# bcgsc/ntSynt

Measured on AMD Instinct MI355X. Metric: minimizer-sketch Gbases/s (sketch with common Bloom filter, inputs resident in HBM), higher is better.
Workload: dtype u64

## Files before the change

ntsynt_amd/csrc/nts_microbench.inc:

```
constexpr int VB_CHAINS = 8;
constexpr int VB_UNROLL = 4;

enum ValuKind
{
  VK_XOR_B32 = 0,
  VK_ALIGNBIT_B32 = 1,
  VK_LSHL_ADD_U64 = 2,
  VK_LSHLREV_B64 = 3,
  VK_MUL_LO_U32 = 4,
  VK_MAD_U64_U32 = 5,
  VK_ADD_CO_PAIR = 6,
  VK_XOR_DEPENDENT = 7,
  VK_ADD3_U32 = 8,
  VK_CMP_ADDC = 9,
  VK_ROLL31_STEP = 10,
  VK_COUNT = 11
};

template <int KIND>
__global__ __launch_bounds__(256) void k_valu_bench(uint32_t iters, unsigned long long* __restrict__ cycles, uint32_t* __restrict__ sink)
{
  uint32_t a[VB_CHAINS];
  uint64_t q[VB_CHAINS];
  const uint32_t seed = threadIdx.x * 2654435761u + blockIdx.x;
#pragma unroll
  for (int c = 0; c < VB_CHAINS; ++c) {
    a[c] = seed + 0x9E3779B9u * (c + 1);
    q[c] = ((uint64_t)a[c] << 32) | (a[c] ^ 0x5bd1e995u);
  }
  const uint32_t b = seed | 1u;
  uint32_t pen = 0;
  const uint64_t b64 = ((uint64_t)b << 20) | 3u;
  __syncthreads();
  const uint64_t t0 = __builtin_amdgcn_s_memtime();
  for (uint32_t it = 0; it < iters; ++it) {
#pragma unroll
    for (int u = 0; u < VB_UNROLL; ++u) {
#pragma unroll
      for (int c = 0; c < VB_CHAINS; ++c) {
        if constexpr (KIND == VK_XOR_B32) asm volatile("v_xor_b32 %0, %1, %0" : "+v"(a[c]) : "v"(b));
        if constexpr (KIND == VK_ALIGNBIT_B32) asm volatile("v_alignbit_b32 %0, %0, %1, 7" : "+v"(a[c]) : "v"(b));
        if constexpr (KIND == VK_LSHL_ADD_U64) asm volatile("v_lshl_add_u64 %0, %0, 1, %1" : "+v"(q[c]) : "v"(b64));
        if constexpr (KIND == VK_LSHLREV_B64) asm volatile("v_lshlrev_b64 %0, 1, %0" : "+v"(q[c]));
        if constexpr (KIND == VK_MUL_LO_U32) asm volatile("v_mul_lo_u32 %0, %0, %1" : "+v"(a[c]) : "v"(b));
        if constexpr (KIND == VK_MAD_U64_U32) asm volatile("v_mad_u64_u32 %0, vcc, %1, %1, %0" : "+v"(q[c]) : "v"(b) : "vcc");
        if constexpr (KIND == VK_ADD_CO_PAIR) {
          uint32_t lo = (uint32_t)q[c], hi = (uint32_t)(q[c] >> 32);
          asm volatile("v_add_co_u32 %0, vcc, %0, %2\n\tv_addc_co_u32 %1, vcc, %1, %2, vcc" : "+v"(lo), "+v"(hi) : "v"(b) : "vcc");
          q[c] = ((uint64_t)hi << 32) | lo;
        }
        if constexpr (KIND == VK_XOR_DEPENDENT) asm volatile("v_xor_b32 %0, %1, %0" : "+v"(a[0]) : "v"(b));
        if constexpr (KIND == VK_ADD3_U32) asm volatile("v_add3_u32 %0, %0, %1, 2" : "+v"(a[c]) : "v"(b));
        if constexpr (KIND == VK_CMP_ADDC)
          asm volatile("v_cmp_ge_u32 vcc, %1, %0\n\tv_addc_co_u32 %0, vcc, %0, %0, vcc" : "+v"(a[c]) : "s"(iters) : "vcc");
        if constexpr (KIND == VK_ROLL31_STEP) {
          uint32_t& wf = a[c & ~1];
          uint32_t& wr = a[c | 1];
          uint32_t s3, t1, x;
          asm volatile("v_add3_u32 %3, %0, %1, 2\n\t"
                       "v_cmp_ge_u32 vcc, %7, %3\n\t"
                       "v_addc_co_u32 %2, vcc, %2, %2, vcc\n\t"
                       "v_lshlrev_b32 %4, 1, %0\n\t"
                       "v_alignbit_b32 %0, %0, %4, 31\n\t"
                       "v_xor_b32 %0, %0, %6\n\t"
                       "v_xor_b32 %5, %1, %6\n\t"
                       "v_lshrrev_b32 %4, 1, %5\n\t"
                       "v_alignbit_b32 %1, %4, %5, 1"
                       : "+v"(wf), "+v"(wr), "+v"(pen), "=&v"(s3), "=&v"(t1), "=&v"(x)
                       : "v"(b), "s"(iters)
                       : "vcc");
        }
      }
    }
  }
  const uint64_t t1 = __builtin_amdgcn_s_memtime();
  uint32_t acc = 0;
#pragma unroll
  for (int c = 0; c < VB_CHAINS; ++c) acc ^= a[c] ^ (uint32_t)q[c] ^ (uint32_t)(q[c] >> 32);
  acc ^= pen;
  if (acc == 0x12345678u) sink[0] = acc;
  if ((threadIdx.x & 63) == 0) cycles[(uint64_t)blockIdx.x * (blockDim.x / 64) + threadIdx.x / 64] = t1 - t0;
}

typedef void (*ValuBenchFn)(uint32_t, unsigned long long*, uint32_t*);
static ValuBenchFn valu_bench_fn(int kind)
{
  switch (kind) {
    case VK_XOR_B32: return k_valu_bench<VK_XOR_B32>;
    case VK_ALIGNBIT_B32: return k_valu_bench<VK_ALIGNBIT_B32>;
    case VK_LSHL_ADD_U64: return k_valu_bench<VK_LSHL_ADD_U64>;
    case VK_LSHLREV_B64: return k_valu_bench<VK_LSHLREV_B64>;
    case VK_MUL_LO_U32: return k_valu_bench<VK_MUL_LO_U32>;
    case VK_MAD_U64_U32: return k_valu_bench<VK_MAD_U64_U32>;
    case VK_ADD_CO_PAIR: return k_valu_bench<VK_ADD_CO_PAIR>;
    case VK_XOR_DEPENDENT: return k_valu_bench<VK_XOR_DEPENDENT>;
    case VK_ADD3_U32: return k_valu_bench<VK_ADD3_U32>;
    case VK_CMP_ADDC: return k_valu_bench<VK_CMP_ADDC>;
    case VK_ROLL31_STEP: return k_valu_bench<VK_ROLL31_STEP>;
  }
  return nullptr;
}
```

ntsynt_amd/csrc/nts_pruned.inc:

```
constexpr uint32_t SEL_CAP = 2048;
constexpr uint32_t SEL_PER_LANE = 64;
constexpr uint32_t SEL_TILE = HASH_THREADS * SEL_PER_LANE;
constexpr uint32_t SPARSE_THREADS = 256;
constexpr uint32_t SPARSE_ITEMS = 2;
constexpr uint32_t SPARSE_BLOCK = SPARSE_THREADS * SPARSE_ITEMS;
constexpr uint32_t CC_TILES = 8;

struct SelParams
{
  const uint8_t* code;
  const uint32_t* pack;
  const uint64_t* run_pos;
  const uint64_t* run_vstart;
  uint32_t n_runs;
  uint64_t n_valid;
  HashParams hp;
  const uint32_t* bf;
  FastMod fm;
  uint64_t tau;
  uint32_t flush_at;
  uint64_t* seg_j;
  uint64_t* seg_key;
  uint64_t seg_cap;
  unsigned long long* seg_count;
// ... 261 lines not shown
    {
      const uint32_t lane = tid & 63u;
      unsigned long long todo = __ballot(shared_lane);
      while (todo) {
        const uint32_t o = (uint32_t)__ffsll((long long)todo) - 1u;
        todo &= todo - 1ULL;
        const uint64_t jo = __shfl(j_lane, (int)o, 64);
        const uint32_t nm = __shfl(n_mine, (int)o, 64);
        const uint32_t run_o = __shfl(run, (int)o, 64);
        const uint32_t cur_o = __shfl(cur, (int)o, 64);
        bool hit = false;
        uint64_t h = 0;
        if (lane < nm) {
          const uint64_t j = jo + lane;
          uint32_t rr = run_o;
          while (P.run_vstart[rr + 1] <= j) ++rr;
          const uint64_t s0 = P.run_pos[rr] + (j - P.run_vstart[rr]);
          uint64_t hf = 0, hr = 0;
          hash_init(P.hp, [&](uint32_t i) { return base_abs(s0 + i); }, hf, hr);
          h = hf + hr;
          hit = (uint32_t)(h >> 32) <= tau_hi;
        }
        const unsigned long long hm = __ballot(hit);
        if (hit) {
          const uint32_t rank = (uint32_t)__popcll(hm & ((1ULL << lane) - 1ULL));
          const uint32_t spare_o = SEL_SLOTS * ROW + (tid - lane + o) * 8u;
          *reinterpret_cast<uint64_t*>(ch_bytes + min(cur_o + rank * ROW, spare_o)) = h;
        }
        if (lane == o) {
          cur += (uint32_t)__popcll(hm) * ROW;
          pen_lo |= (uint32_t)hm;
          pen_hi |= (uint32_t)(hm >> 32);
        }
      }
    }
    if (!over) flush();
    if (!__syncthreads_or(over)) {
      static_assert(SEL_SLOTS * HASH_THREADS >= SEL_CAP, "the general path stages SEL_CAP candidates in the same arrays");
      uint32_t accepted = 0;
      const uint32_t off = block_excl_scan_256(acc, s_w, &accepted);
      if (tid == 0) {
        s_base = accepted ? atomicAdd(&P.seg_count[seg], (unsigned long long)accepted) : 0ULL;
        P.tile_off[tile] = s_base;
        P.tile_cnt[tile] = accepted;
        P.tile_ordered[tile] = 1;
      }
      __syncthreads();
      const uint64_t base = s_base;
      if (accepted == 0 || base + accepted > P.seg_cap) return;
      uint64_t* dj = P.seg_j + (uint64_t)seg * P.seg_cap + base + off;
      uint64_t* dk = P.seg_key + (uint64_t)seg * P.seg_cap + base + off;
      for (uint32_t i = 0; i < acc; ++i) {
        dj[i] = J0 + first + (uint32_t)__builtin_ctzll(acc_mask);
        acc_mask &= acc_mask - 1;
        dk[i] = s_ch[i * HASH_THREADS + tid];
      }
      return;
    }
  }
  if (tid == 0) P.tile_ordered[tile] = 0;
  roll_pass(0, SEL_TILE);
  __syncthreads();
  const uint32_t total = s_ctl[0];
  if (total <= SEL_CAP) {
    uint32_t mine = 0, accepted = 0;
    const uint32_t bits = probe_staged(total, &mine);
    (void)block_excl_scan_256(mine, s_w, &accepted);
    if (tid == 0) {
      s_base = accepted ? atomicAdd(&P.seg_count[seg], (unsigned long long)accepted) : 0ULL;
      P.tile_off[tile] = s_base;
      P.tile_cnt[tile] = accepted;
    }
    __syncthreads();
    const uint64_t base = s_base;
    if (accepted == 0 || base + accepted > P.seg_cap) return;
    write_staged(total, bits, (uint64_t)seg * P.seg_cap + base);
    return;
  }
  constexpr uint32_t RANGE = 2048;
  uint32_t accepted = 0;
  for (uint32_t r0 = 0; r0 < SEL_TILE; r0 += RANGE) {
    __syncthreads();
    if (tid == 0) s_ctl[0] = 0;
    __syncthreads();
    roll_pass(r0, r0 + RANGE);
    __syncthreads();
    uint32_t mine = 0, acc = 0;
    (void)probe_staged(s_ctl[0], &mine);
    (void)block_excl_scan_256(mine, s_w, &acc);
    accepted += acc;
  }
  if (tid == 0) {
    s_base = accepted ? atomicAdd(&P.seg_count[seg], (unsigned long long)accepted) : 0ULL;
    P.tile_off[tile] = s_base;
    P.tile_cnt[tile] = accepted;
    s_ctl[1] = 0;
  }
  __syncthreads();
  const uint64_t base = s_base;
  if (accepted == 0 || base + accepted > P.seg_cap) return;
  for (uint32_t r0 = 0; r0 < SEL_TILE; r0 += RANGE) {
    __syncthreads();
    if (tid == 0) s_ctl[0] = 0;
    __syncthreads();
    roll_pass(r0, r0 + RANGE);
    __syncthreads();
    uint32_t mine = 0;
    const uint32_t n = s_ctl[0];
    const uint32_t bits = probe_staged(n, &mine);
    write_staged(n, bits, (uint64_t)seg * P.seg_cap + base);
  }
}

constexpr uint32_t HIW_TILE = 64 * SEL_PER_LANE;
constexpr uint32_t HIW_WAVES = 8;
constexpr uint32_t HIW_THREADS = 64 * HIW_WAVES;
constexpr uint32_t HIW_PER_MAX = 4;
constexpr uint32_t HI_K_MAX = 32;

__device__ __forceinline__ uint32_t hi_wform(uint64_t h)
{
  const uint32_t hi = (uint32_t)(h >> 32);
  return (hi & ~1u) | (hi >> 31);
}

__device__ __forceinline__ uint64_t sload64(const uint64_t* p, uint32_t idx)
{
  uint64_t v;
  asm volatile("s_load_dwordx2 %0, %1, %2\n\ts_waitcnt lgkmcnt(0)" : "=&s"(v) : "s"(p), "s"(idx * 8u) : "memory");
  return v;
}

__device__ __forceinline__ uint32_t wave_excl_scan_small(uint32_t v, uint64_t below, uint32_t* total)
{
  uint32_t pre = 0, tot = 0;
#pragma unroll
  for (uint32_t b = 0; b < 3; ++b) {
    const unsigned long long m = __ballot((v >> b) & 1u);
    pre += (uint32_t)__popcll(m & below) << b;
    tot += (uint32_t)__popcll(m) << b;
  }
  if (__ballot(v >> 3) != 0ULL) {
#pragma unroll
    for (uint32_t b = 3; b < 7; ++b) {
      const unsigned long long m = __ballot((v >> b) & 1u);
      pre += (uint32_t)__popcll(m & below) << b;
      tot += (uint32_t)__popcll(m) << b;
    }
  }
  *total = tot;
  return pre;
}

__device__ __forceinline__ void hi_roll64(const uint32_t (&ro)[5], const uint32_t (&ri)[5], uint32_t sh_o, uint32_t sh_i, const ulonglong2* s_T,
                                          const uint2* s_roll, uint32_t nch, uint32_t limit, uint32_t& pen0, uint32_t& pen1)
{
  uint32_t O[4], I[4];
#pragma unroll
  for (int q = 0; q < 4; ++q) {
    O[q] = __builtin_amdgcn_alignbit(ro[q + 1], ro[q], sh_o);
    I[q] = __builtin_amdgcn_alignbit(ri[q + 1], ri[q], sh_i);
  }
  uint32_t wf = 0, wr = 0;
#pragma unroll
  for (uint32_t c = 0; c < HI_K_MAX / 4; ++c) {
    if (c < nch) {
      const ulonglong2 e = s_T[c * 256u + ((O[c >> 2] >> (8u * (c & 3u))) & 255u)];
      wf ^= (uint32_t)(e.x >> 32);
      wr ^= (uint32_t)(e.y >> 32);
    }
  }
  wf = (wf & ~1u) | (wf >> 31);
  wr = (wr & ~1u) | (wr >> 31);
  const uint8_t* const roll_bytes = reinterpret_cast<const uint8_t*>(s_roll);
  pen0 = pen1 = 0;
#pragma unroll
  for (int q = 0; q < 4; ++q) {
    const uint32_t even = (O[q] & 0x33333333u) | ((I[q] & 0x33333333u) << 2);
    const uint32_t odd = ((O[q] >> 2) & 0x33333333u) | (I[q] & 0xCCCCCCCCu);
    uint32_t pen = 0;
#pragma unroll
    for (int j0 = 0; j0 < 16; j0 += 8) {
      uint2 tb[8];
#pragma unroll
      for (int jj = 0; jj < 8; ++jj) {
        const int j = j0 + jj;
        const uint32_t pairs = (j & 1) ? odd : even;
        const int sh = 4 * (j >> 1) - 3;
        const uint32_t t8 = (sh < 0 ? pairs << 3 : pairs >> sh) & 0x78u;
        tb[jj] = *reinterpret_cast<const uint2*>(roll_bytes + t8);
      }
#pragma unroll
      for (int jj = 0; jj < 8; ++jj) {
        const uint32_t s = wf + wr + 2u;
        asm("v_cmp_ge_u32 vcc, %2, %1\n\tv_addc_co_u32 %0, vcc, %0, %0, vcc" : "+v"(pen) : "v"(s), "s"(limit) : "vcc");
        wf = __builtin_amdgcn_alignbit(wf, wf << 1, 31) ^ tb[jj].x;
        const uint32_t x = wr ^ tb[jj].y;
        wr = __builtin_amdgcn_alignbit(x >> 1, x, 1);
      }
    }
    const uint32_t nat = __brev(pen) >> 16;
    if (q < 2)
      pen0 |= nat << (16 * q);
    else
      pen1 |= nat << (16 * (q - 2));
  }
}

__device__ __forceinline__ uint2 hi_roll_multirun(const uint32_t* pack, const uint64_t* run_pos, const uint64_t* run_vstart, uint32_t n_runs,
                                               uint32_t run_lo, uint64_t j_lane, uint32_t n_mine, uint32_t k, const ulonglong2* s_T,
                                               const uint2* s_roll, uint32_t nch, uint32_t limit, bool& straddles)
{
  uint32_t rl = run_lo, rh = n_runs;
  while (rh - rl > 1) {
    const uint32_t mid = rl + ((rh - rl) >> 1);
    if (run_vstart[mid] <= j_lane)
      rl = mid;
    else
      rh = mid;
  }
  uint32_t pen0, pen1;
  straddles = false;
  if (n_mine == SEL_PER_LANE && j_lane + SEL_PER_LANE <= run_vstart[rl + 1]) {
    const uint64_t xo = run_pos[rl] + (j_lane - run_vstart[rl]);
    const uint32_t* wo = pack + (xo >> 4);
    const uint32_t* wi = pack + ((xo + k) >> 4);
    uint32_t ro[5], ri[5];
#pragma unroll
    for (int q = 0; q < 5; ++q) {
      ro[q] = wo[q];
      ri[q] = wi[q];
    }
    hi_roll64(ro, ri, 2u * ((uint32_t)xo & 15u), 2u * ((uint32_t)(xo + k) & 15u), s_T, s_roll, nch, limit, pen0, pen1);
  } else {
    pen0 = pen1 = 0;
    straddles = true;
  }
  return make_uint2(pen0, pen1);
}

constexpr uint32_t HIW_STAGE_WORDS = 272;
constexpr uint32_t ELIM_REACH = 6;

template <bool HAS_BF, uint32_t HIW_PER>
__global__ __launch_bounds__(HIW_THREADS) void k_hash_select_hi(SelParams P, uint32_t nch, uint32_t tpw, uint64_t n_tiles)
{
  constexpr uint32_t HIW_LIST = 64 * HIW_PER;
  static_assert(HIW_PER == 2 || HIW_PER == 4, "the waits count the probes");
  extern __shared__ __align__(16) uint8_t hi_dyn_lds[];
  ulonglong2* const s_T = reinterpret_cast<ulonglong2*>(hi_dyn_lds);
  __shared__ uint2 s_roll[16];
  __shared__ __align__(16) uint32_t s_stage[HIW_WAVES][2][HIW_STAGE_WORDS];
  __shared__ uint16_t s_lists[HIW_WAVES][HIW_LIST];
  __shared__ __align__(16) uint32_t s_probe[HIW_WAVES][HIW_PER][64];
  const uint32_t tid = threadIdx.x, lane = tid & 63u;
  const uint32_t wv = __builtin_amdgcn_readfirstlane(tid >> 6);
  {
    const ulonglong2* src = reinterpret_cast<const ulonglong2*>(P.hp.init4);
    for (uint32_t i = tid; i < nch * 256u; i += HIW_THREADS) s_T[i] = src[i];
  }
  if (tid < 16) s_roll[tid] = make_uint2(hi_wform(P.hp.roll_f[tid]), hi_wform(P.hp.roll_r[tid]));
  __syncthreads();
  uint16_t* const s_list = s_lists[wv];
  const uint32_t stage_lds = (uint32_t)(uintptr_t)(__attribute__((address_space(3))) uint32_t*)(&s_stage[wv][0][0]);
  const uint32_t probe_lds = (uint32_t)(uintptr_t)(__attribute__((address_space(3))) uint32_t*)(&s_probe[wv][0][0]);
  const uint32_t k = P.hp.k;
  const uint32_t tau_hi = (uint32_t)(P.tau >> 32);
  const uint32_t limit = 2u * (tau_hi >> 1) + 4u;
  const uint32_t key16_shift = 48u - (uint32_t)__builtin_clzll(P.tau | 0x10000ULL);
  const uint32_t blk = (blockIdx.x & 1u) ? gridDim.x - 1u - (blockIdx.x >> 1) : (blockIdx.x >> 1);
  const uint64_t tile_first = ((uint64_t)blk * HIW_WAVES + wv) * tpw;
  if (tile_first >= n_tiles) return;
  const uint32_t my_tiles = (uint32_t)min((uint64_t)tpw, n_tiles - tile_first);
  const uint32_t first = SEL_PER_LANE * lane;
  const uint64_t below = (1ULL << lane) - 1ULL;

  uint32_t run_next = 0;
  {
    const uint64_t J0 = tile_first * HIW_TILE;
    uint32_t lo = 0, hi = P.n_runs;
    while (hi - lo > 1) {
      const uint32_t mid = lo + ((hi - lo) >> 1);
      if (sload64(P.run_vstart, mid) <= J0)
        lo = mid;
      else
        hi = mid;
    }
    run_next = lo;
  }
  auto geometry = [&](uint64_t tile, uint64_t& J0, uint64_t& P0, uint32_t& len, uint32_t& run, uint32_t& single) {
    J0 = tile * HIW_TILE;
    len = (uint32_t)min((uint64_t)HIW_TILE, P.n_valid - J0);
    uint64_t v1 = sload64(P.run_vstart, run_next + 1);
    while (v1 <= J0) {
      ++run_next;
      v1 = sload64(P.run_vstart, run_next + 1);
    }
    run = run_next;
    single = J0 + len <= v1 ? 1u : 0u;
    P0 = sload64(P.run_pos, run_next) + (J0 - sload64(P.run_vstart, run_next));
  };
  uint32_t run_end = P.n_runs;
  auto position_of = [&](uint64_t j, uint32_t run_lo) -> uint64_t {
    uint32_t rl = run_lo, rh = run_end;
    while (rh - rl > 1) {
      const uint32_t mid = rl + ((rh - rl) >> 1);
      if (P.run_vstart[mid] <= j)
        rl = mid;
      else
        rh = mid;
    }
    return P.run_pos[rl] + (j - P.run_vstart[rl]);
  };
  auto stage_dma = [&](uint64_t t_P0, bool real, uint32_t buf) {
    const uint64_t w0 = real ? ((t_P0 >> 4) & ~3ULL) : 0ULL;
    const uint32_t lds = stage_lds + buf * (HIW_STAGE_WORDS * 4u);
    const uint32_t* ga = P.pack + w0 + 4u * lane;
    asm volatile("s_mov_b32 m0, %1\n\ts_nop 0\n\tglobal_load_lds_dwordx4 %0, off" ::"v"(ga), "s"(lds) : "memory");
    if (lane < 4) {
      const uint32_t* gb = ga + 256;
      asm volatile("s_mov_b32 m0, %1\n\ts_nop 0\n\tglobal_load_lds_dwordx4 %0, off" ::"v"(gb), "s"(lds + 1024u) : "memory");
    }
  };
  auto full_hash = [&](const uint32_t* words, uint32_t sh) -> uint64_t {
    const uint32_t w0 = words[0], w1 = words[1], w2 = words[2];
    const uint32_t b_lo = __builtin_amdgcn_alignbit(w1, w0, sh), b_hi = __builtin_amdgcn_alignbit(w2, w1, sh);
    uint64_t f = 0, r = 0;
#pragma unroll
    for (uint32_t c = 0; c < HI_K_MAX / 4; ++c) {
      if (c < nch) {
        const ulonglong2 e = s_T[c * 256u + (((c < 4 ? b_lo : b_hi) >> (8u * (c & 3u))) & 255u)];
        f ^= e.x;
        r ^= e.y;
      }
    }
    return f + r;
  };

  uint64_t pd_h[HIW_PER];
  uint32_t pd_i[HIW_PER], pd_w[HIW_PER], pd_b[HIW_PER];
  uint32_t pd_m = 0;
  uint64_t pd_tile = ~0ULL, pd_J0 = 0;
  uint32_t pd_single = 0;
#pragma unroll
  for (uint32_t i = 0; i < HIW_PER; ++i) {
    pd_h[i] = 0;
    pd_i[i] = 0;
    pd_w[i] = 0;
    pd_b[i] = 0;
  }
  auto issue_probes = [&]() {
    if (HAS_BF) {
      const uint32_t* wp[HIW_PER];
#pragma unroll
      for (uint32_t i = 0; i < HIW_PER; ++i) {
        const uint64_t bidx = P.fm(pd_h[i]);
        pd_b[i] = (uint32_t)bidx & 31u;
        wp[i] = P.bf + (((pd_m >> i) & 1u) ? (bidx >> 5) : 0ULL);
      }
#pragma unroll
      for (uint32_t i = 0; i < HIW_PER; ++i)
        asm volatile("s_mov_b32 m0, %1\n\ts_nop 0\n\tglobal_load_lds_dword %0, off" ::"v"(wp[i]), "s"(probe_lds + i * 256u) : "memory");
    }
  };
  auto wait_stage = [&]() {
    if (HAS_BF && HIW_PER == 4)
      asm volatile("s_waitcnt vmcnt(6)" ::: "memory");
    else if (HAS_BF)
      asm volatile("s_waitcnt vmcnt(4)" ::: "memory");
    else
      asm volatile("s_waitcnt vmcnt(2)" ::: "memory");
  };
  auto wait_probes = [&]() {
    if (HAS_BF) {
      asm volatile("s_waitcnt vmcnt(0)" ::: "memory");
#pragma unroll
      for (uint32_t i = 0; i < HIW_PER; ++i) pd_w[i] = s_probe[wv][i][lane];
    }
  };
  uint32_t wave_run = 0;
  auto finish_pending = [&]() {
    if (pd_tile == ~0ULL) return;
    uint32_t okm = pd_m;
    if (HAS_BF) {
#pragma unroll
      for (uint32_t i = 0; i < HIW_PER; ++i)
        if (!((pd_w[i] >> pd_b[i]) & 1u)) okm &= ~(1u << i);
    }
    uint32_t rank = 0, accepted = 0;
#pragma unroll
    for (uint32_t i = 0; i < HIW_PER; ++i) {
      const unsigned long long bm = __ballot((okm >> i) & 1u);
      rank += (uint32_t)__popcll(bm & below);
      accepted += (uint32_t)__popcll(bm);
    }
    if (P.w_elim && pd_single && accepted > 2u && accepted + 2u * ELIM_REACH <= HIW_LIST) {
      uint32_t* const s_e = &s_probe[wv][0][0];
      if (lane < 2u * ELIM_REACH) s_e[lane < ELIM_REACH ? lane : accepted + lane] = 0xFFFFFFFFu;
      uint32_t n = 0;
#pragma unroll
      for (uint32_t i = 0; i < HIW_PER; ++i) {
        if ((okm >> i) & 1u) {
          s_e[ELIM_REACH + rank + n] = ((uint32_t)(pd_h[i] >> key16_shift) << 16) | pd_i[i];
          ++n;
        }
      }
      __builtin_amdgcn_fence(__ATOMIC_RELEASE, "wavefront");
      __builtin_amdgcn_wave_barrier();
      __builtin_amdgcn_fence(__ATOMIC_ACQUIRE, "wavefront");
      unsigned long long lost[HIW_PER];
#pragma unroll
      for (uint32_t ps = 0; ps < HIW_PER; ++ps) {
        lost[ps] = 0ULL;
        if (64u * ps < accepted) {
// ... 1343 lines not shown
```

ntsynt_amd/csrc/ntsynt_hip.hip:

```cpp
#include "nts_internal.h"

namespace {


__global__ __launch_bounds__(256) void k_encode(uint8_t* __restrict__ buf, uint64_t n)
{
  const uint64_t i = ((uint64_t)blockIdx.x * blockDim.x + threadIdx.x) * 16;
  if (i >= n) return;
  if (i + 16 <= n) {
    uint4 v = *reinterpret_cast<const uint4*>(buf + i);
    uint32_t wds[4] = { v.x, v.y, v.z, v.w };
#pragma unroll
    for (int q = 0; q < 4; ++q) {
      uint32_t out = 0;
#pragma unroll
      for (int b = 0; b < 4; ++b) {
        uint32_t c = (wds[q] >> (8 * b)) & 0xFFu;
        c &= 0xDFu;
        uint32_t code = (c == 'A') ? 0u : (c == 'C') ? 1u : (c == 'G') ? 2u : (c == 'T' || c == 'U') ? 3u : 4u;
        out |= code << (8 * b);
      }
      wds[q] = out;
    }
    *reinterpret_cast<uint4*>(buf + i) = make_uint4(wds[0], wds[1], wds[2], wds[3]);
// ... 2194 lines not shown
  if (!ctx || !genome_bf || !repeat_bf || !g || k == 0) return fail(ctx, NTS_EINVAL, "nts_bf_insert_repeats: bad arguments");
  if (genome_bf->bytes != repeat_bf->bytes) return fail(ctx, NTS_EINVAL, "nts_bf_insert_repeats: filters differ in size");
  genome_bf->popcnt = -1;
  ++genome_bf->version;
  repeat_bf->popcnt = -1;
  ++repeat_bf->version;
  HIP_TRY(ctx, hipSetDevice(ctx->device));
  GenomeTables scratch;
  const GenomeTables* T = nullptr;
  int rc = get_tables(ctx, g, k, nullptr, 0, scratch, &T);
  if (rc) return rc;
  rc = launch_hash<MODE_REPEAT>(ctx, "bf_repeats", g, *T, k, genome_bf, repeat_bf, nullptr);
  if (rc) return rc;
  HIP_TRY(ctx, hipStreamSynchronize(ctx->stream));
  return NTS_OK;
}

int nts_bf_build_mode(nts_ctx* ctx, int mode)
{
  if (!ctx || mode < 0 || mode > 2) return fail(ctx, NTS_EINVAL, "nts_bf_build_mode: mode must be 0 (auto), 1 (atomic) or 2 (binned)");
  ctx->bf_build_mode = mode;
  return NTS_OK;
}

int nts_bf_insert(nts_ctx* ctx, nts_bf* bf, const nts_genome* g, uint32_t k)
{
  return bf_hash_pass(ctx, nullptr, bf, g, k);
}

int nts_bf_cascade(nts_ctx* ctx, const nts_bf* prev, nts_bf* next, const nts_genome* g, uint32_t k)
{
  if (!prev) return fail(ctx, NTS_EINVAL, "nts_bf_cascade: prev is NULL");
  return bf_hash_pass(ctx, prev, next, g, k);
}

int nts_bf_and(nts_ctx* ctx, nts_bf* acc, const nts_bf* other)
{
  if (!ctx || !acc || !other || acc->bytes != other->bytes) return fail(ctx, NTS_EINVAL, "nts_bf_and: filters differ in size");
  acc->popcnt = -1;
  ++acc->version;
  HIP_TRY(ctx, hipSetDevice(ctx->device));
  const uint64_t n16 = (acc->bytes + 15) / 16;
  const uint32_t blocks = (uint32_t)std::min<uint64_t>((n16 + 255) / 256, 256 * 8);
  ScopedTimer t(ctx, "bf_and");
  NTS_LAUNCH(k_bf_and, dim3(blocks), dim3(256), 0, ctx->stream, (uint4*)acc->d_words, (const uint4*)other->d_words, n16);
  HIP_TRY(ctx, hipGetLastError());
  return NTS_OK;
}

int nts_bf_popcount(nts_ctx* ctx, const nts_bf* bf, uint64_t* bits_set)
{
  if (!ctx || !bf || !bits_set) return fail(ctx, NTS_EINVAL, "nts_bf_popcount: bad arguments");
  if (bf->popcnt >= 0 && bf->owned) {
    *bits_set = (uint64_t)bf->popcnt;
    return NTS_OK;
  }
  HIP_TRY(ctx, hipSetDevice(ctx->device));
  unsigned long long* d = (unsigned long long*)ws_get(ctx, "popcnt", 64);
  if (!d) return NTS_ENOMEM;
  hipMemsetAsync(d, 0, sizeof(unsigned long long), ctx->stream);
  const uint64_t n16 = (bf->bytes + 15) / 16;
  const uint32_t blocks = (uint32_t)std::min<uint64_t>((n16 + 255) / 256, 256 * 8);
  {
    ScopedTimer t(ctx, "bf_popcount");
    NTS_LAUNCH(k_bf_popcount, dim3(blocks), dim3(256), 0, ctx->stream, (const uint4*)bf->d_words, n16, d);
  }
  unsigned long long h = 0;
  hipMemcpyAsync(&h, d, sizeof(h), hipMemcpyDeviceToHost, ctx->stream);
  hipError_t e = hipStreamSynchronize(ctx->stream);
  if (e != hipSuccess) return fail(ctx, NTS_EHIP, std::string("popcount: ") + hipGetErrorString(e));
  bf->popcnt = (int64_t)h;
  *bits_set = h;
  return NTS_OK;
}

int nts_bench_random_probe(nts_ctx* ctx, const nts_bf* bf, uint64_t n_probes, uint32_t repeats, double* avg_ms, uint64_t* hits)
{
  if (!ctx || !bf || !avg_ms || n_probes == 0 || repeats == 0) return fail(ctx, NTS_EINVAL, "nts_bench_random_probe: bad arguments");
  HIP_TRY(ctx, hipSetDevice(ctx->device));
  unsigned long long* d = (unsigned long long*)ws_get(ctx, "bench_sink", 8);
  if (!d) return NTS_ENOMEM;
  HIP_TRY(ctx, hipMemsetAsync(d, 0, 8, ctx->stream));
  const FastMod fm = make_fastmod(bf->bytes * 8);
  const uint64_t blocks = (n_probes + 8191) / 8192;
  if (blocks > 0x7FFFFFFFULL) return fail(ctx, NTS_ERANGE, "nts_bench_random_probe: too many probes");
  hipEvent_t a, b;
  hipEventCreate(&a);
  hipEventCreate(&b);
  NTS_LAUNCH(k_bench_probe, dim3((uint32_t)blocks), dim3(256), 0, ctx->stream, bf->d_words, fm, n_probes, (uint64_t)1, d);
  hipEventRecord(a, ctx->stream);
  for (uint32_t r = 0; r < repeats; ++r)
    NTS_LAUNCH(k_bench_probe, dim3((uint32_t)blocks), dim3(256), 0, ctx->stream, bf->d_words, fm, n_probes, (uint64_t)(r + 2), d);
  hipEventRecord(b, ctx->stream);
  unsigned long long h = 0;
  hipMemcpyAsync(&h, d, 8, hipMemcpyDeviceToHost, ctx->stream);
  hipError_t e = hipStreamSynchronize(ctx->stream);
  float ms = 0;
  hipEventElapsedTime(&ms, a, b);
  hipEventDestroy(a);
  hipEventDestroy(b);
  if (e != hipSuccess) return fail(ctx, NTS_EHIP, std::string("bench: ") + hipGetErrorString(e));
  *avg_ms = ms / repeats;
  if (hits) *hits = h;
  return NTS_OK;
}

int nts_mod_indices(nts_ctx* ctx, uint64_t bits, int form, const uint64_t* h, uint64_t n, uint64_t* out)
{
  if (!ctx || bits < 2 || !h || !out || form < -1 || form > 2) return fail(ctx, NTS_EINVAL, "nts_mod_indices: bad arguments");
  if (n == 0) return NTS_OK;
  HIP_TRY(ctx, hipSetDevice(ctx->device));
  uint64_t* d = (uint64_t*)ws_get(ctx, "mod_idx", n * 8);
  if (!d) return NTS_ENOMEM;
  FastMod fm = make_fastmod(bits);
  if (form >= 0) fm.form = std::min<uint32_t>(fm.form, (uint32_t)form);
  HIP_TRY(ctx, hipMemcpyAsync(d, h, n * 8, hipMemcpyHostToDevice, ctx->stream));
  NTS_LAUNCH(k_mod_indices, dim3((uint32_t)std::min<uint64_t>((n + 255) / 256, 65535)), dim3(256), 0, ctx->stream, d, n, fm);
  HIP_TRY(ctx, hipGetLastError());
  HIP_TRY(ctx, hipMemcpyAsync(out, d, n * 8, hipMemcpyDeviceToHost, ctx->stream));
  HIP_TRY(ctx, hipStreamSynchronize(ctx->stream));
  return NTS_OK;
}

int nts_bench_valu(nts_ctx* ctx, int kind, uint32_t waves_per_simd, uint32_t iters, double* wall_ms, double* cycles_per_instr,
                   double* instr_per_wave)
{
  if (!ctx || kind < 0 || kind >= VK_COUNT || waves_per_simd == 0 || waves_per_simd > 8 || iters == 0)
    return fail(ctx, NTS_EINVAL, "nts_bench_valu: bad arguments");
  HIP_TRY(ctx, hipSetDevice(ctx->device));
  hipDeviceProp_t prop;
  HIP_TRY(ctx, hipGetDeviceProperties(&prop, ctx->device));
  const uint32_t cus = (uint32_t)prop.multiProcessorCount;
  const uint32_t blocks = cus * waves_per_simd;
  const uint64_t n_waves = (uint64_t)blocks * 4;
  unsigned long long* d_cyc = (unsigned long long*)ws_get(ctx, "valu_cycles", n_waves * 8);
  uint32_t* d_sink = (uint32_t*)ws_get(ctx, "valu_sink", 64);
  if (!d_cyc || !d_sink) return NTS_ENOMEM;
  ValuBenchFn fn = valu_bench_fn(kind);
  hipEvent_t a, b;
  hipEventCreate(&a);
  hipEventCreate(&b);
  NTS_LAUNCH(fn, dim3(blocks), dim3(256), 0, ctx->stream, iters / 8 + 1, d_cyc, d_sink);
  hipEventRecord(a, ctx->stream);
  NTS_LAUNCH(fn, dim3(blocks), dim3(256), 0, ctx->stream, iters, d_cyc, d_sink);
  hipEventRecord(b, ctx->stream);
  std::vector<unsigned long long> cyc(n_waves);
  hipMemcpyAsync(cyc.data(), d_cyc, n_waves * 8, hipMemcpyDeviceToHost, ctx->stream);
  hipError_t e = hipStreamSynchronize(ctx->stream);
  float ms = 0;
  hipEventElapsedTime(&ms, a, b);
  hipEventDestroy(a);
  hipEventDestroy(b);
  if (e != hipSuccess) return fail(ctx, NTS_EHIP, std::string("nts_bench_valu: ") + hipGetErrorString(e));
  const double per_iter = (double)VB_CHAINS * VB_UNROLL * (kind == VK_ADD_CO_PAIR || kind == VK_CMP_ADDC ? 2 : kind == VK_ROLL31_STEP ? 9 : 1);
  const double n_instr = per_iter * iters;
  std::sort(cyc.begin(), cyc.end());
  const double median = (double)cyc[n_waves / 2];
  if (wall_ms) *wall_ms = ms;
  if (cycles_per_instr) *cycles_per_instr = median / (n_instr * waves_per_simd);
  if (instr_per_wave) *instr_per_wave = n_instr;
  return NTS_OK;
}

int nts_bf_download(nts_ctx* ctx, const nts_bf* bf, uint8_t* host, uint64_t bytes)
{
  if (!ctx || !bf || !host || bytes != bf->bytes) return fail(ctx, NTS_EINVAL, "nts_bf_download: size mismatch");
  HIP_TRY(ctx, hipSetDevice(ctx->device));
  hipEvent_t ready;
  HIP_TRY(ctx, hipEventCreateWithFlags(&ready, hipEventDisableTiming));
  hipError_t e = hipEventRecord(ready, ctx->stream);
  if (e == hipSuccess) e = hipStreamWaitEvent(ctx->copy_stream, ready, 0);
  if (e == hipSuccess) e = hipMemcpyAsync(host, bf->d_words, bytes, hipMemcpyDeviceToHost, ctx->copy_stream);
  if (e == hipSuccess) e = hipStreamSynchronize(ctx->copy_stream);
  hipEventDestroy(ready);
  HIP_TRY(ctx, e);
  return NTS_OK;
}

int nts_bf_upload(nts_ctx* ctx, nts_bf* bf, const uint8_t* host, uint64_t bytes)
{
  if (!ctx || !bf || !host || bytes != bf->bytes) return fail(ctx, NTS_EINVAL, "nts_bf_upload: size mismatch");
  bf->popcnt = -1;
  ++bf->version;
  HIP_TRY(ctx, hipSetDevice(ctx->device));
  HIP_TRY(ctx, hipMemcpyAsync(bf->d_words, host, bytes, hipMemcpyHostToDevice, ctx->stream));
  HIP_TRY(ctx, hipStreamSynchronize(ctx->stream));
  return NTS_OK;
}

int nts_bf_save(nts_ctx* ctx, const nts_bf* bf, const char* path, const void* header, uint64_t header_bytes, uint32_t n_threads)
{
  if (!ctx || !bf || !path || (header_bytes && !header)) return fail(ctx, NTS_EINVAL, "nts_bf_save: bad arguments");
  HIP_TRY(ctx, hipSetDevice(ctx->device));
  hipEvent_t ready;
  HIP_TRY(ctx, hipEventCreateWithFlags(&ready, hipEventDisableTiming));
  HIP_TRY(ctx, hipEventRecord(ready, ctx->stream));
  const int fd = open(path, O_CREAT | O_TRUNC | O_RDWR, 0644);
  if (fd < 0) {
    hipEventDestroy(ready);
    return fail(ctx, NTS_EINVAL, std::string("nts_bf_save: cannot create ") + path);
  }
  auto write_at = [fd](const void* src, uint64_t len, uint64_t at) {
    const uint8_t* p = (const uint8_t*)src;
    while (len) {
      const ssize_t got = pwrite(fd, p, len, (off_t)at);
      if (got <= 0) return false;
      p += got;
      at += (uint64_t)got;
      len -= (uint64_t)got;
    }
    return true;
  };
  bool ok = header_bytes == 0 || write_at(header, header_bytes, 0);
  std::atomic<uint64_t> next(0);
  std::atomic<bool> failed(false);
  const uint64_t CHUNK = IO_CHUNK;
  const uint64_t n_chunks = (bf->bytes + CHUNK - 1) / CHUNK;
  const uint8_t* src = (const uint8_t*)bf->d_words;
  const int device = ctx->device;
  const unsigned T = ok ? io_lanes(ctx, ctx->io_down, (unsigned)std::max<uint64_t>(1, std::min<uint64_t>(n_threads ? n_threads : 6, (n_chunks + 7) / 8))) : 0;
  if (ok && T == 0) ok = false;
  auto worker = [&](unsigned lane) {
    if (hipSetDevice(device) != hipSuccess) {
      failed.store(true);
      return;
    }
    nts_ctx::IoLane& io = ctx->io_down[lane];
    hipStream_t st = io.stream;
    uint8_t* const* stage = io.stage;
    if (hipStreamWaitEvent(st, ready, 0) != hipSuccess) {
      failed.store(true);
      return;
    }
    uint64_t cur = next.fetch_add(1), cur_len = 0;
    int slot = 0;
    if (cur < n_chunks) {
      cur_len = std::min(CHUNK, bf->bytes - cur * CHUNK);
      if (hipMemcpyAsync(stage[slot], src + cur * CHUNK, cur_len, hipMemcpyDeviceToHost, st) != hipSuccess) failed.store(true);
    }
    while (cur < n_chunks && !failed.load()) {
      if (hipStreamSynchronize(st) != hipSuccess) {
        failed.store(true);
        break;
      }
      const uint64_t nxt = next.fetch_add(1);
      uint64_t nxt_len = 0;
      if (nxt < n_chunks) {
        nxt_len = std::min(CHUNK, bf->bytes - nxt * CHUNK);
        if (hipMemcpyAsync(stage[slot ^ 1], src + nxt * CHUNK, nxt_len, hipMemcpyDeviceToHost, st) != hipSuccess) failed.store(true);
      }
      if (!write_at(stage[slot], cur_len, header_bytes + cur * CHUNK)) failed.store(true);
      cur = nxt;
      cur_len = nxt_len;
      slot ^= 1;
    }
    hipStreamSynchronize(st);
  };
  if (ok) {
    std::vector<std::thread> pool;
    for (unsigned t = 0; t < T; ++t) pool.emplace_back(worker, t);
    for (auto& th : pool) th.join();
  }
  close(fd);
  hipEventDestroy(ready);
  if (!ok || failed.load()) return fail(ctx, NTS_EHIP, std::string("nts_bf_save: writing ") + path + " failed");
  return NTS_OK;
}

int nts_hash_all(nts_ctx* ctx, const nts_genome* g, uint32_t k, uint64_t** h0, uint64_t* n_out)
{
  if (!ctx || !g || !h0 || !n_out || k == 0) return fail(ctx, NTS_EINVAL, "nts_hash_all: bad arguments");
  HIP_TRY(ctx, hipSetDevice(ctx->device));
  GenomeTables scratch;
  const GenomeTables* T = nullptr;
  int rc = get_tables(ctx, g, k, nullptr, 0, scratch, &T);
  if (rc) return rc;
  const RunTable& rt = T->rt;
  uint64_t* d_keys = nullptr;
  uint64_t* d_lin = nullptr;
  HIP_TRY(ctx, dev_malloc((void**)&d_keys, key_buffer_elems(rt.n_valid) * 8));
  HIP_TRY(ctx, dev_malloc((void**)&d_lin, std::max<uint64_t>(rt.n_valid, 1) * 8));
  rc = launch_hash<MODE_KEYS>(ctx, "hash_only", g, *T, k, nullptr, nullptr, d_keys);
  uint64_t* host = (uint64_t*)malloc(std::max<uint64_t>(rt.n_valid, 1) * 8);
  if (rc == NTS_OK && rt.n_valid) {
    NTS_LAUNCH(k_keys_linear, dim3((uint32_t)((rt.n_valid + 255) / 256)), dim3(256), 0, ctx->stream, d_keys, rt.n_valid, d_lin);
    hipMemcpyAsync(host, d_lin, rt.n_valid * 8, hipMemcpyDeviceToHost, ctx->stream);
  }
  hipError_t e = hipStreamSynchronize(ctx->stream);
  dev_free(d_keys);
  dev_free(d_lin);
  if (rc != NTS_OK || e != hipSuccess) {
    free(host);
    return rc != NTS_OK ? rc : fail(ctx, NTS_EHIP, std::string("hash_all: ") + hipGetErrorString(e));
  }
  *h0 = host;
  *n_out = rt.n_valid;
  return NTS_OK;
}

int nts_minhash(nts_ctx* ctx, const nts_genome* g, uint32_t k, uint32_t s, uint64_t* out, uint32_t* n_out)
{
  if (!ctx || !g || !out || !n_out || k == 0 || s == 0) return fail(ctx, NTS_EINVAL, "nts_minhash: bad arguments");
  HIP_TRY(ctx, hipSetDevice(ctx->device));
  return minhash_run(ctx, g, k, s, out, n_out);
}

}
// ... 1451 lines not shown
```

ntsynt_amd/device.py:

```python
import ctypes
import os

import numpy as np

from . import _lib
from ._lib import Interval, c_vp, u64


class NtsError(RuntimeError):
    pass


MEM_EVENT_NAMES = ("driver_calls", "ns_in_driver_calls", "served_from_cache", "retried_after_emptying_the_cache", "bytes_from_driver",
                   "bytes_to_driver", "ns_waiting_for_device_before_keeping_a_block", "reserve_calls")


def mem_events(lib):
    out = (ctypes.c_uint64 * 8)()
    lib.nts_mem_events(out)
    return dict(zip(MEM_EVENT_NAMES, [int(x) for x in out]))


def mem_events_since(lib, before):
    now = mem_events(lib)
    d = {k: now[k] - before[k] for k in now}
    return {"hipMalloc_hipFree_calls": d["driver_calls"], "ms_in_hipMalloc_hipFree": round(d["ns_in_driver_calls"] * 1e-6, 2),
            "allocations_served_from_kept_memory": d["served_from_cache"], "allocations_retried_after_emptying_the_cache": d["retried_after_emptying_the_cache"],
            "GB_from_driver": round(d["bytes_from_driver"] / 1e9, 3), "GB_to_driver": round(d["bytes_to_driver"] / 1e9, 3),
            "ms_waiting_for_device_before_keeping_a_block": round(d["ns_waiting_for_device_before_keeping_a_block"] * 1e-6, 2),
            "reserve_calls": d["reserve_calls"]}


class Context:

    def __init__(self, device=0, variant=None):
        self.lib = _lib.load(variant)
        self.variant = variant
        h = c_vp()
        rc = self.lib.nts_init(int(device), ctypes.byref(h))
        if rc != 0:
            raise NtsError(f"nts_init({device}) failed: {self.lib.nts_last_error(None).decode()} "
                           "(a real MI355X is required; there is no CPU fallback)")
        self.h = h
        self.device = int(device)

    def check(self, rc, what=""):
        if rc != 0:
            raise NtsError(f"{what}: {self.lib.nts_last_error(self.h).decode()} (code {rc})")

    def sync(self):
        self.check(self.lib.nts_sync(self.h), "nts_sync")

    def profile(self, enable=True):
        level = int(enable) if not isinstance(enable, bool) else (1 if enable else 0)
        self.check(self.lib.nts_profile(self.h, level), "nts_profile")

    def timing(self, name):
        ms, n = ctypes.c_double(), u64()
        self.check(self.lib.nts_timing(self.h, name.encode(), ctypes.byref(ms), ctypes.byref(n)), "nts_timing")
        return ms.value, n.value

    def sketch_mode(self, mode="auto", prune_c=0):
        code = {"auto": 0, "dense": 1, "pruned": 2}[mode]
        self.check(self.lib.nts_sketch_mode(self.h, code, int(prune_c)), "nts_sketch_mode")
        self._sketch_mode = (mode, int(prune_c))

    def sketch_summary(self, mode=None):
        last = ctypes.c_uint32()
        code = {None: -1, "auto": 0, "never": 1, "no-lds": 2}[mode]
        self.check(self.lib.nts_sketch_summary(self.h, code, ctypes.byref(last)), "nts_sketch_summary")
        return last.value

    def sketch_select(self, impl="auto"):
        self.check(self.lib.nts_sketch_select(self.h, {"auto": 0, "full": 1, "hi": 2}[impl]), "nts_sketch_select")

    def sketch_tiers(self, mode=None, x0=0.0, half_steps=False):
        a, b, c = u64(), u64(), ctypes.c_uint32()
        code = {None: -1, "auto": 0, "never": 1, "always": 2}[mode]
        self.check(self.lib.nts_sketch_tiers(self.h, code, float(x0), int(bool(half_steps)), ctypes.byref(a), ctypes.byref(b), ctypes.byref(c)),
                   "nts_sketch_tiers")
        return a.value, b.value, c.value

    def bf_build_mode(self, mode="auto"):
        self.check(self.lib.nts_bf_build_mode(self.h, {"auto": 0, "atomic": 1, "binned": 2}[mode]), "nts_bf_build_mode")

    def sketch_stats(self):
        a, b, c, d = u64(), u64(), u64(), ctypes.c_uint32()
        self.check(self.lib.nts_sketch_stats(self.h, ctypes.byref(a), ctypes.byref(b), ctypes.byref(c), ctypes.byref(d)),
                   "nts_sketch_stats")
        self.last_prune_c = d.value
        return a.value, b.value, c.value

    def path_stats(self):
        a, b, c = u64(), u64(), ctypes.c_uint32()
        self.check(self.lib.nts_path_stats(self.h, ctypes.byref(a), ctypes.byref(b), ctypes.byref(c)), "nts_path_stats")
        return {"sketch_many_listed": a.value, "bf_direct_indices": b.value, "bf_list_fallback": c.value}

    def bf_level_stats(self):
        a, b = ctypes.c_uint32(), u64()
        self.check(self.lib.nts_bf_level_stats(self.h, ctypes.byref(a), ctypes.byref(b)), "nts_bf_level_stats")
        return {"sparse_level": a.value, "accepted_kmers": b.value}

    VALU_KINDS = ["v_xor_b32", "v_alignbit_b32", "v_lshl_add_u64", "v_lshlrev_b64", "v_mul_lo_u32", "v_mad_u64_u32",
                  "v_add_co_u32+v_addc_co_u32", "v_xor_b32 (dependent chain)", "v_add3_u32", "v_cmp_ge_u32+v_addc_co_u32",
                  "roll31 step (9 instructions)"]

    def bench_valu(self, kind, waves_per_simd=4, iters=20000):
        ms, cyc, n = ctypes.c_double(), ctypes.c_double(), ctypes.c_double()
        k = self.VALU_KINDS.index(kind) if isinstance(kind, str) else int(kind)
        self.check(self.lib.nts_bench_valu(self.h, k, int(waves_per_simd), int(iters), ctypes.byref(ms), ctypes.byref(cyc),
                                           ctypes.byref(n)), "nts_bench_valu")
        per_cu = 4 * waves_per_simd * n.value / (ms.value * 1e-3)
        return {"instruction": self.VALU_KINDS[k], "waves_per_simd": int(waves_per_simd), "wall_ms": round(ms.value, 4),
                "cycles_per_wave_instr_per_simd": round(cyc.value, 3), "wave_instr_per_s_per_cu": per_cu,
                "implied_clock_GHz": round(per_cu * cyc.value / 4 / 1e9, 3)}

    def set_graph_budget(self, nbytes):
        self.check(self.lib.nts_graph_budget(self.h, int(nbytes)), "nts_graph_budget")

    def graph_last_plan(self):
        v, e, o, p = ctypes.c_uint32(), ctypes.c_uint32(), ctypes.c_uint32(), u64()
        self.check(self.lib.nts_graph_last_plan(self.h, ctypes.byref(v), ctypes.byref(e), ctypes.byref(p), ctypes.byref(o)),
                   "nts_graph_last_plan")
        return {"v_slices": v.value, "e_slices": e.value, "scratch_peak": p.value, "oversize": o.value}

    def mem_stats(self):
        a, b, c, d = u64(), u64(), u64(), u64()
        self.check(self.lib.nts_mem_stats(self.h, ctypes.byref(a), ctypes.byref(b), ctypes.byref(c), ctypes.byref(d)), "nts_mem_stats")
        return {"live": a.value, "peak": b.value, "device_used": c.value, "device_total": d.value}

    def alloc_stats(self):
        n, ms = u64(), ctypes.c_double()
        self.lib.nts_alloc_stats(ctypes.byref(n), ctypes.byref(ms))
        return n.value, ms.value

    def mem_trim(self):
        return int(self.lib.nts_mem_trim())

    def mem_cache_stats(self):
        a, b = u64(), u64()
        self.lib.nts_mem_cache_stats(ctypes.byref(a), ctypes.byref(b))
        return a.value, b.value

    def mem_reset_peak(self):
        self.lib.nts_mem_reset_peak()

    def mem_reserve(self, nbytes):
        got = u64()
        self.check(self.lib.nts_mem_reserve(self.device, int(nbytes), ctypes.byref(got)), "nts_mem_reserve")
        return got.value

    def mem_reserve_async(self, nbytes):
        import threading
        box = {"got": 0}

        def work():
            try:
                box["got"] = self.mem_reserve(nbytes)
            except Exception:
                box["got"] = 0
        th = threading.Thread(target=work, name="nts_mem_reserve", daemon=True)
        th.start()

        class _Pending:
            def join(self_inner):
                th.join()
                return box["got"]
        return _Pending()

    def mem_events(self):
        return mem_events(self.lib)

    def mem_events_since(self, before):
        return mem_events_since(self.lib, before)

    def trim_ingest(self):
        self.check(self.lib.nts_ingest_trim(self.h), "nts_ingest_trim")

    def trim_bf_build(self):
        self.check(self.lib.nts_bf_build_trim(self.h), "nts_bf_build_trim")

    def close(self):
        if self.h:
            self.lib.nts_destroy(self.h)
            self.h = None

    def __del__(self):
        try:
            self.close()
        except Exception:
            pass


BF_ROUNDING = {"up": 0, "down": 1, "none": 2}


def bf_size_bytes(genome_bp, fpr, rounding="up"):
    a, c = u64(), u64()
    rc = _lib.load().nts_bf_size_bytes_ex(int(genome_bp), float(fpr), BF_ROUNDING[rounding], ctypes.byref(a), ctypes.byref(c))
    if rc != 0:
        raise NtsError("nts_bf_size_bytes: bad arguments")
    return a.value, c.value


class Genome:

    def __init__(self, ctx, names, seq, rec_off, rec_len):
        self.ctx = ctx
        self.names = list(names)
        seq = np.ascontiguousarray(seq, dtype=np.uint8)
        self.rec_off = np.ascontiguousarray(rec_off, dtype=np.uint64)
        self.rec_len = np.ascontiguousarray(rec_len, dtype=np.uint64)
        self.n_bytes = int(seq.size)
        h = c_vp()
        ctx.check(ctx.lib.nts_genome_upload(ctx.h, seq.ctypes.data, seq.size,
                                            self.rec_off.ctypes.data_as(_lib.c_u64p),
                                            self.rec_len.ctypes.data_as(_lib.c_u64p),
                                            len(self.names), ctypes.byref(h)), "nts_genome_upload")
        self.h = h

    @classmethod
    def synth(cls, ctx, total_bp, n_contigs, seed_ancestor, seed_genome, substitution_rate):
        g = cls.__new__(cls)
        g.ctx = ctx
        per = int(total_bp) // int(n_contigs)
        g.names = [f"chr{i + 1}" for i in range(n_contigs)]
        g.rec_len = np.full(n_contigs, per, dtype=np.uint64)
        g.rec_off = (np.arange(n_contigs, dtype=np.uint64) * np.uint64(per)).astype(np.uint64)
        g.n_bytes = per * int(n_contigs)
        h = c_vp()
        ctx.check(ctx.lib.nts_genome_synth(ctx.h, int(total_bp), int(n_contigs), int(seed_ancestor), int(seed_genome),
                                           float(substitution_rate), ctypes.byref(h)), "nts_genome_synth")
        g.h = h
        return g

    @classmethod
    def synth_plan(cls, ctx, plan, seed_ancestor, seed_genome, substitution_rate, rep=None, names=None):
        rec_len, pieces = plan[0], plan[1]
        g = cls.__new__(cls)
        g.ctx = ctx
        rec_len = np.ascontiguousarray(rec_len, dtype=np.uint64)
        pieces = np.ascontiguousarray(pieces)
        assert pieces.dtype.itemsize == 32
        g.names = list(names) if names is not None else [f"chr{i + 1}" for i in range(rec_len.size)]
        g.rec_len = rec_len
        g.rec_off = np.concatenate(([0], np.cumsum(rec_len[:-1]))).astype(np.uint64)
        g.n_bytes = int(rec_len.sum())
        h = c_vp()
        rp = None
        if rep is not None:
            rp = _lib.SynthRepeats(**{k_: int(v) for k_, v in rep.items()})
        ctx.check(ctx.lib.nts_genome_synth_plan_ex(ctx.h, rec_len.size, rec_len.ctypes.data, pieces.size, pieces.ctypes.data,
                                                   int(seed_ancestor), int(seed_genome), float(substitution_rate),
                                                   ctypes.byref(rp) if rp is not None else None, ctypes.byref(h)),
                  "nts_genome_synth_plan")
        g.h = h
        return g

# ... 383 lines not shown
```

Before: 1500.

## Software-pipeline roll table fetches in hi_roll64 with explicit LDS waits

Restructures the 64-step rolling hash penalty loop in hi_roll64 into batches of four, prefetching the next batch's LDS table entries into a double buffer and waiting on lgkmcnt with sched barriers, so LDS latency overlaps the dependent VALU chain. The roll table is widened to 16-byte entries so the index can be computed with a single SDWA byte-select AND instead of shift-and-mask. A microbenchmark kind for the fetch-plus-step sequence is also added. The hand-placed waitcnt and sched barriers constrain the compiler scheduler and rely on exact LDS op counts, and the wider table uses more LDS.

Measured after the change: 1504, median of 6. About the same (+0.3%).

```diff
diff --git a/ntsynt_amd/csrc/nts_microbench.inc b/ntsynt_amd/csrc/nts_microbench.inc
--- a/ntsynt_amd/csrc/nts_microbench.inc
+++ b/ntsynt_amd/csrc/nts_microbench.inc
@@ -14,7 +14,8 @@
   VK_ADD3_U32 = 8,
   VK_CMP_ADDC = 9,
   VK_ROLL31_STEP = 10,
-  VK_COUNT = 11
+  VK_ROLL31_FETCH = 11,
+  VK_COUNT = 12
 };
 
 template <int KIND>
@@ -31,6 +32,10 @@
   const uint32_t b = seed | 1u;
   uint32_t pen = 0;
   const uint64_t b64 = ((uint64_t)b << 20) | 3u;
+  __shared__ uint4 s_roll[KIND == VK_ROLL31_FETCH ? 16 : 1];
+  if constexpr (KIND == VK_ROLL31_FETCH) {
+    if (threadIdx.x < 16) s_roll[threadIdx.x] = make_uint4(seed, ~seed, 0u, 0u);
+  }
   __syncthreads();
   const uint64_t t0 = __builtin_amdgcn_s_memtime();
   for (uint32_t it = 0; it < iters; ++it) {
@@ -53,6 +58,15 @@
         if constexpr (KIND == VK_ADD3_U32) asm volatile("v_add3_u32 %0, %0, %1, 2" : "+v"(a[c]) : "v"(b));
         if constexpr (KIND == VK_CMP_ADDC)
           asm volatile("v_cmp_ge_u32 vcc, %1, %0\n\tv_addc_co_u32 %0, vcc, %0, %0, vcc" : "+v"(a[c]) : "s"(iters) : "vcc");
+        if constexpr (KIND == VK_ROLL31_FETCH) {
+          if (c == 0) {
+            const uint32_t ro[5] = {a[0], a[1], a[2], a[3], a[4]}, ri[5] = {a[3], a[4], a[5], a[6], a[7]};
+            uint32_t p0, p1;
+            hi_roll64(ro, ri, 2u * (b & 15u), 2u * ((b >> 4) & 15u), nullptr, s_roll, 0u, iters, p0, p1);
+            a[u & 7] += p0;
+            a[(u + 4) & 7] ^= p1;
+          }
+        }
         if constexpr (KIND == VK_ROLL31_STEP) {
           uint32_t& wf = a[c & ~1];
           uint32_t& wr = a[c | 1];
@@ -97,6 +111,7 @@
     case VK_ADD3_U32: return k_valu_bench<VK_ADD3_U32>;
     case VK_CMP_ADDC: return k_valu_bench<VK_CMP_ADDC>;
     case VK_ROLL31_STEP: return k_valu_bench<VK_ROLL31_STEP>;
+    case VK_ROLL31_FETCH: return k_valu_bench<VK_ROLL31_FETCH>;
   }
   return nullptr;
 }
diff --git a/ntsynt_amd/csrc/nts_pruned.inc b/ntsynt_amd/csrc/nts_pruned.inc
--- a/ntsynt_amd/csrc/nts_pruned.inc
+++ b/ntsynt_amd/csrc/nts_pruned.inc
@@ -437,8 +437,23 @@
   return pre;
 }
 
+__device__ __forceinline__ uint32_t hi_byte_and(uint32_t v, uint32_t mask, int byte)
+{
+  uint32_t r;
+  switch (byte) {
+  case 0: asm("v_and_b32_sdwa %0, %1, %2 dst_sel:DWORD dst_unused:UNUSED_PAD src0_sel:DWORD src1_sel:BYTE_0" : "=v"(r) : "s"(mask), "v"(v)); break;
+  case 1: asm("v_and_b32_sdwa %0, %1, %2 dst_sel:DWORD dst_unused:UNUSED_PAD src0_sel:DWORD src1_sel:BYTE_1" : "=v"(r) : "s"(mask), "v"(v)); break;
+  case 2: asm("v_and_b32_sdwa %0, %1, %2 dst_sel:DWORD dst_unused:UNUSED_PAD src0_sel:DWORD src1_sel:BYTE_2" : "=v"(r) : "s"(mask), "v"(v)); break;
+  default: asm("v_and_b32_sdwa %0, %1, %2 dst_sel:DWORD dst_unused:UNUSED_PAD src0_sel:DWORD src1_sel:BYTE_3" : "=v"(r) : "s"(mask), "v"(v)); break;
+  }
+  return r;
+}
+
+constexpr int HI_ROLL_BATCH = 4;
+#define HI_WAIT_LGKM(n) (0xC07F | ((n) << 8))
+
 __device__ __forceinline__ void hi_roll64(const uint32_t (&ro)[5], const uint32_t (&ri)[5], uint32_t sh_o, uint32_t sh_i, const ulonglong2* s_T,
-                                          const uint2* s_roll, uint32_t nch, uint32_t limit, uint32_t& pen0, uint32_t& pen1)
+                                          const uint4* s_roll, uint32_t nch, uint32_t limit, uint32_t& pen0, uint32_t& pen1)
 {
   uint32_t O[4], I[4];
 #pragma unroll
@@ -458,43 +473,60 @@
   wf = (wf & ~1u) | (wf >> 31);
   wr = (wr & ~1u) | (wr >> 31);
   const uint8_t* const roll_bytes = reinterpret_cast<const uint8_t*>(s_roll);
-  pen0 = pen1 = 0;
-#pragma unroll
-  for (int q = 0; q < 4; ++q) {
+  const uint32_t nib_hi = 0xF0u;
+  auto fetch = [&](int b, uint2 (&tb)[HI_ROLL_BATCH]) {
+    const int q = (b * HI_ROLL_BATCH) >> 4;
     const uint32_t even = (O[q] & 0x33333333u) | ((I[q] & 0x33333333u) << 2);
     const uint32_t odd = ((O[q] >> 2) & 0x33333333u) | (I[q] & 0xCCCCCCCCu);
-    uint32_t pen = 0;
-#pragma unroll
-    for (int j0 = 0; j0 < 16; j0 += 8) {
-      uint2 tb[8];
-#pragma unroll
-      for (int jj = 0; jj < 8; ++jj) {
-        const int j = j0 + jj;
-        const uint32_t pairs = (j & 1) ? odd : even;
-        const int sh = 4 * (j >> 1) - 3;
-        const uint32_t t8 = (sh < 0 ? pairs << 3 : pairs >> sh) & 0x78u;
-        tb[jj] = *reinterpret_cast<const uint2*>(roll_bytes + t8);
-      }
-#pragma unroll
-      for (int jj = 0; jj < 8; ++jj) {
-        const uint32_t s = wf + wr + 2u;
-        asm("v_cmp_ge_u32 vcc, %2, %1\n\tv_addc_co_u32 %0, vcc, %0, %0, vcc" : "+v"(pen) : "v"(s), "s"(limit) : "vcc");
-        wf = __builtin_amdgcn_alignbit(wf, wf << 1, 31) ^ tb[jj].x;
-        const uint32_t x = wr ^ tb[jj].y;
-        wr = __builtin_amdgcn_alignbit(x >> 1, x, 1);
-      }
-    }
-    const uint32_t nat = __brev(pen) >> 16;
-    if (q < 2)
-      pen0 |= nat << (16 * q);
-    else
-      pen1 |= nat << (16 * (q - 2));
+    const uint32_t even4 = even << 4, odd4 = odd << 4;
+#pragma unroll
+    for (int jj = 0; jj < HI_ROLL_BATCH; ++jj) {
+      const int j = ((b * HI_ROLL_BATCH) & 15) + jj;
+      const int n = j >> 1;
+      const uint32_t pairs = (n & 1) ? ((j & 1) ? odd : even) : ((j & 1) ? odd4 : even4);
+      const uint32_t t16 = hi_byte_and(pairs, nib_hi, n >> 1);
+      tb[jj] = *reinterpret_cast<const uint2*>(roll_bytes + t16);
+    }
+  };
+  constexpr int N_BATCH = 64 / HI_ROLL_BATCH;
+  uint2 tb[2][HI_ROLL_BATCH];
+  fetch(0, tb[0]);
+  pen0 = pen1 = 0;
+  uint32_t pen = 0;
+#pragma unroll
+  for (int b = 0; b < N_BATCH; ++b) {
+    if (b + 1 < N_BATCH) {
+      fetch(b + 1, tb[(b + 1) & 1]);
+      __builtin_amdgcn_sched_barrier(0);
+      __builtin_amdgcn_s_waitcnt(HI_WAIT_LGKM(HI_ROLL_BATCH));
+    } else {
+      __builtin_amdgcn_sched_barrier(0);
+      __builtin_amdgcn_s_waitcnt(HI_WAIT_LGKM(0));
+    }
+    __builtin_amdgcn_sched_barrier(0);
+#pragma unroll
+    for (int jj = 0; jj < HI_ROLL_BATCH; ++jj) {
+      const uint32_t s = wf + wr + 2u;
+      asm("v_cmp_ge_u32 vcc, %2, %1\n\tv_addc_co_u32 %0, vcc, %0, %0, vcc" : "+v"(pen) : "v"(s), "s"(limit) : "vcc");
+      wf = __builtin_amdgcn_alignbit(wf, wf << 1, 31) ^ tb[b & 1][jj].x;
+      const uint32_t x = wr ^ tb[b & 1][jj].y;
+      wr = __builtin_amdgcn_alignbit(x >> 1, x, 1);
+    }
+    if (((b + 1) * HI_ROLL_BATCH & 15) == 0) {
+      const int q = (b * HI_ROLL_BATCH) >> 4;
+      const uint32_t nat = __brev(pen) >> 16;
+      if (q < 2)
+        pen0 |= nat << (16 * q);
+      else
+        pen1 |= nat << (16 * (q - 2));
+      pen = 0;
+    }
   }
 }
 
 __device__ __forceinline__ uint2 hi_roll_multirun(const uint32_t* pack, const uint64_t* run_pos, const uint64_t* run_vstart, uint32_t n_runs,
                                                uint32_t run_lo, uint64_t j_lane, uint32_t n_mine, uint32_t k, const ulonglong2* s_T,
-                                               const uint2* s_roll, uint32_t nch, uint32_t limit, bool& straddles)
+                                               const uint4* s_roll, uint32_t nch, uint32_t limit, bool& straddles)
 {
   uint32_t rl = run_lo, rh = n_runs;
   while (rh - rl > 1) {
@@ -534,7 +566,7 @@
   static_assert(HIW_PER == 2 || HIW_PER == 4, "the waits count the probes");
   extern __shared__ __align__(16) uint8_t hi_dyn_lds[];
   ulonglong2* const s_T = reinterpret_cast<ulonglong2*>(hi_dyn_lds);
-  __shared__ uint2 s_roll[16];
+  __shared__ uint4 s_roll[16];
   __shared__ __align__(16) uint32_t s_stage[HIW_WAVES][2][HIW_STAGE_WORDS];
   __shared__ uint16_t s_lists[HIW_WAVES][HIW_LIST];
   __shared__ __align__(16) uint32_t s_probe[HIW_WAVES][HIW_PER][64];
@@ -544,7 +576,7 @@
     const ulonglong2* src = reinterpret_cast<const ulonglong2*>(P.hp.init4);
     for (uint32_t i = tid; i < nch * 256u; i += HIW_THREADS) s_T[i] = src[i];
   }
-  if (tid < 16) s_roll[tid] = make_uint2(hi_wform(P.hp.roll_f[tid]), hi_wform(P.hp.roll_r[tid]));
+  if (tid < 16) s_roll[tid] = make_uint4(hi_wform(P.hp.roll_f[tid]), hi_wform(P.hp.roll_r[tid]), 0u, 0u);
   __syncthreads();
   uint16_t* const s_list = s_lists[wv];
   const uint32_t stage_lds = (uint32_t)(uintptr_t)(__attribute__((address_space(3))) uint32_t*)(&s_stage[wv][0][0]);
diff --git a/ntsynt_amd/csrc/ntsynt_hip.hip b/ntsynt_amd/csrc/ntsynt_hip.hip
--- a/ntsynt_amd/csrc/ntsynt_hip.hip
+++ b/ntsynt_amd/csrc/ntsynt_hip.hip
@@ -2370,7 +2370,8 @@
   hipEventDestroy(a);
   hipEventDestroy(b);
   if (e != hipSuccess) return fail(ctx, NTS_EHIP, std::string("nts_bench_valu: ") + hipGetErrorString(e));
-  const double per_iter = (double)VB_CHAINS * VB_UNROLL * (kind == VK_ADD_CO_PAIR || kind == VK_CMP_ADDC ? 2 : kind == VK_ROLL31_STEP ? 9 : 1);
+  const double per_iter = kind == VK_ROLL31_FETCH ? (double)VB_UNROLL * 64 * 11
+                                                  : (double)VB_CHAINS * VB_UNROLL * (kind == VK_ADD_CO_PAIR || kind == VK_CMP_ADDC ? 2 : kind == VK_ROLL31_STEP ? 9 : 1);
   const double n_instr = per_iter * iters;
   std::sort(cyc.begin(), cyc.end());
   const double median = (double)cyc[n_waves / 2];
diff --git a/ntsynt_amd/device.py b/ntsynt_amd/device.py
--- a/ntsynt_amd/device.py
+++ b/ntsynt_amd/device.py
@@ -103,7 +103,7 @@
 
     VALU_KINDS = ["v_xor_b32", "v_alignbit_b32", "v_lshl_add_u64", "v_lshlrev_b64", "v_mul_lo_u32", "v_mad_u64_u32",
                   "v_add_co_u32+v_addc_co_u32", "v_xor_b32 (dependent chain)", "v_add3_u32", "v_cmp_ge_u32+v_addc_co_u32",
-                  "roll31 step (9 instructions)"]
+                  "roll31 step (9 instructions)", "roll31 step with table fetch (11 instructions)"]
 
     def bench_valu(self, kind, waves_per_simd=4, iters=20000):
         ms, cyc, n = ctypes.c_double(), ctypes.c_double(), ctypes.c_double()
```
